# zhufengGNSS/gnss-sdr-1

Measured on AMD Instinct MI355X. Metric: Msamples/s tracked (N-channel multicorrelator, whole job), higher is better.
Workload: dtype f32

## Files before the change

gnss-sdr-1_amd/csrc/trk_closed_loop.hip:

```cpp
#include "gc_internal.h"
#include <algorithm>
#include <cstddef>
#include <cstdlib>
#include "gc_stream.h"
#include "trk_loop_device.hpp"
#include <cstring>
#include <vector>

template <int NTAPS, int THREADS, int FMT, bool DATA, bool HD = false>
__global__ __launch_bounds__(THREADS) void trk_closed_loop_kernel(LoopChan* __restrict__ chans,
    gc_loop_record* __restrict__ recs, int n_epochs, int lds_table_floats, const unsigned long long* __restrict__ limits, int resident)
{
    extern __shared__ float lds[];
    __shared__ LoopChan s;
    __shared__ gc_epoch_params s_p;
    __shared__ float2 s_corr[GC_MAX_TAPS];
    __shared__ int s_go;
    const int ch = blockIdx.x;
    const int tid = threadIdx.x;
    {
        const unsigned* src = reinterpret_cast<const unsigned*>(&chans[ch]);
        unsigned* dst = reinterpret_cast<unsigned*>(&s);
        for (unsigned i = tid; i < sizeof(LoopChan) / 4; i += THREADS) dst[i] = src[i];
    }
    __syncthreads();
    if (s.n_taps != NTAPS)
        {
            for (int e = 0; e < n_epochs; e++)
                {
                    unsigned* w = reinterpret_cast<unsigned*>(&recs[(size_t)ch * n_epochs + e]);
                    for (unsigned i = tid; i < sizeof(gc_loop_record) / 4; i += THREADS) w[i] = 0u;
                }
            return;
        }
    const unsigned long long limit = limits ? limits[ch] : s.chan.n_iq;
    loop_periods<NTAPS, THREADS, FMT, DATA, HD>(s, s_p, s_corr, s_go, lds, &recs[(size_t)ch * n_epochs], n_epochs, lds_table_floats, limit, resident);
    __syncthreads();
    {
        unsigned* dst = reinterpret_cast<unsigned*>(&chans[ch]);
        const unsigned* src = reinterpret_cast<const unsigned*>(&s);
        for (unsigned i = tid; i < sizeof(LoopChan) / 4; i += THREADS) dst[i] = src[i];
    }
}

#ifdef GNSSCORR_EXPERIMENTS
#ifndef LOOP_SLICE_FENCES
#define LOOP_SLICE_FENCES 0
#endif
struct LoopPrep
{
    gc_epoch_params p;
    int go;
    int pad;
};

template <bool HD>
__global__ __launch_bounds__(64) void trk_loop_prepare_kernel(LoopChan* __restrict__ chans, LoopPrep* __restrict__ prep, gc_loop_record* __restrict__ recs, int n_epochs,
    const unsigned long long* __restrict__ limits)
{
    __shared__ LoopChan s;
    __shared__ gc_epoch_params s_p;
    const int ch = blockIdx.x, tid = threadIdx.x;
    {
        const unsigned* src = reinterpret_cast<const unsigned*>(&chans[ch]);
        unsigned* dst = reinterpret_cast<unsigned*>(&s);
        for (unsigned i = tid; i < sizeof(LoopChan) / 4; i += 64) dst[i] = src[i];
    }
    __syncthreads();
    if (s.n_taps == 0) return;
    if (tid == 0)
        {
            const unsigned long long limit = limits ? limits[ch] : s.chan.n_iq;
            const int go = loop_prepare<HD>(s, limit, s_p, &recs[(size_t)ch * n_epochs]);
            prep[ch].p = s_p;
            prep[ch].go = go;
        }
    __syncthreads();
    {
        unsigned* dst = reinterpret_cast<unsigned*>(&chans[ch]);
        const unsigned* src = reinterpret_cast<const unsigned*>(&s);
        for (unsigned i = tid; i < sizeof(LoopChan) / 4; i += 64) dst[i] = src[i];
    }
}

template <int NTAPS, int THREADS, int FMT, bool DATA, bool HD>
__global__ __launch_bounds__(THREADS) void trk_closed_loop_slice_kernel(LoopChan* __restrict__ chans, gc_loop_record* __restrict__ recs, int n_epochs, int e,
    int n_channels, int n_slices, int lds_table_floats, const unsigned long long* __restrict__ limits, LoopPrep* __restrict__ prep, float2* __restrict__ partial,
    unsigned* __restrict__ tickets)
{
    extern __shared__ float lds[];
    __shared__ LoopChan s;
    __shared__ gc_epoch_params s_p;
    __shared__ float2 s_corr[GC_MAX_TAPS];
    __shared__ int s_go, s_last;
    const int tid = threadIdx.x;
    const int x = blockIdx.x & 7, q = blockIdx.x >> 3;
    const int slice = q % n_slices, ch = (q / n_slices) * 8 + x;
    if (ch >= n_channels) return;
    constexpr int NOUT = NTAPS + (DATA ? 1 : 0);
    gc_loop_record* rec = &recs[(size_t)ch * n_epochs + e];
    if (tid == 0)
        {
            s.chan = chans[ch].chan;
            s.n_taps = chans[ch].n_taps;
            s_p = prep[ch].p;
            s_go = prep[ch].go;
        }
    __syncthreads();
    if (s.n_taps != NTAPS)
        {
            if (slice == 0)
                {
                    unsigned* w = reinterpret_cast<unsigned*>(rec);
                    for (unsigned i = tid; i < sizeof(gc_loop_record) / 4; i += THREADS) w[i] = 0u;
                }
            return;
        }
    if (s_go)
        {
            const float2 r = trk_epoch<NTAPS, HD, HD, FMT, false, false, THREADS, DATA, LOOP_PF, false, LOOP_NT != 0, LOOP_WHOLE != 0>(s.chan, s_p, slice, n_slices, lds_table_floats, lds, LOOP_ALIGN_PAIRS);
            if (tid < NOUT) s_corr[tid] = r;
        }
    __syncthreads();
    if (tid == 0)
        {
            float* pv = reinterpret_cast<float*>(partial + ((size_t)ch * n_slices + slice) * GC_MAX_TAPS);
            if (s_go)
                for (int t = 0; t < NOUT; t++)
                    {
                        __hip_atomic_store(pv + 2 * t, s_corr[t].x, __ATOMIC_RELAXED, __HIP_MEMORY_SCOPE_AGENT);
                        __hip_atomic_store(pv + 2 * t + 1, s_corr[t].y, __ATOMIC_RELAXED, __HIP_MEMORY_SCOPE_AGENT);
                    }
#if LOOP_SLICE_FENCES
            __builtin_amdgcn_fence(__ATOMIC_RELEASE, "agent");
#endif
            asm volatile("s_waitcnt vmcnt(0)" ::: "memory");
            const unsigned ticket = __hip_atomic_fetch_add(tickets + ch, 1u, __ATOMIC_RELAXED, __HIP_MEMORY_SCOPE_AGENT);
            s_last = (ticket == (unsigned)n_slices - 1u) ? 1 : 0;
#if LOOP_SLICE_FENCES
            if (s_last) __builtin_amdgcn_fence(__ATOMIC_ACQUIRE, "agent");
#endif
        }
    __syncthreads();
    if (!s_last) return;
    {
        const unsigned* src = reinterpret_cast<const unsigned*>(&chans[ch]);
        unsigned* dst = reinterpret_cast<unsigned*>(&s);
        for (unsigned i = tid; i < sizeof(LoopChan) / 4; i += THREADS) dst[i] = src[i];
    }
    __syncthreads();
    if (tid == 0)
        {
            const unsigned long long limit = limits ? limits[ch] : s.chan.n_iq;
            if (s_go)
                {
                    float2 taps[GC_MAX_TAPS];
                    for (int t = 0; t < NOUT; t++) taps[t] = make_float2(0.f, 0.f);
                    for (int sl = 0; sl < n_slices; sl++)
                        {
                            const float* qv = reinterpret_cast<const float*>(partial + ((size_t)ch * n_slices + sl) * GC_MAX_TAPS);
                            for (int t = 0; t < NOUT; t++)
                                {
                                    taps[t].x += __hip_atomic_load(qv + 2 * t, __ATOMIC_RELAXED, __HIP_MEMORY_SCOPE_AGENT);
                                    taps[t].y += __hip_atomic_load(qv + 2 * t + 1, __ATOMIC_RELAXED, __HIP_MEMORY_SCOPE_AGENT);
                                }
                        }
                    for (int t = 0; t < NOUT; t++) s_corr[t] = taps[t];
                    loop_after_correlation<NTAPS, DATA>(s, s_corr, rec);
                }
            if (e + 1 < n_epochs)
                {
                    const int go = loop_prepare<HD>(s, limit, s_p, rec + 1);
                    prep[ch].p = s_p;
                    prep[ch].go = go;
                }
            __hip_atomic_store(tickets + ch, 0u, __ATOMIC_RELAXED, __HIP_MEMORY_SCOPE_AGENT);
        }
    __syncthreads();
    {
        unsigned* dst = reinterpret_cast<unsigned*>(&chans[ch]);
        const unsigned* src = reinterpret_cast<const unsigned*>(&s);
        for (unsigned i = tid; i < sizeof(LoopChan) / 4; i += THREADS) dst[i] = src[i];
    }
}

#else
struct LoopPrep;
#endif

__global__ void trk_loop_start_kernel(LoopChan* chans, int ch)
{
    if (threadIdx.x == 0 && blockIdx.x == 0) loop_start(chans[ch]);
}

struct gc_trk_loop
{
    gc_ctx* ctx = nullptr;
    gc_ctx_ref ctx_ref;
    int n_channels = 0, max_code_len = 0, n_taps = 0;
    LoopChan* d_chans = nullptr;
    float* d_codes = nullptr;
    float* d_data_codes = nullptr;
    std::vector<LoopSync> sync;
    std::vector<int> data_code_len;
    int pilot = -1;
    int high_dyn = 0;
    int mixed = 0;
    std::vector<int> code_len;
    std::vector<char> track_pilot;
    gc_loop_record* d_recs = nullptr;
    size_t recs_cap = 0;
    int forced_threads = 0;
    int forced_slices = 0;
    LoopPrep* d_prep = nullptr;
    float2* d_slice_partial = nullptr;
    unsigned* d_tickets = nullptr;
    int slice_cap = 0;
    int iq_format = GC_IQ_F32;
    std::vector<char> started;
    std::vector<const void*> iq;
    std::vector<unsigned long long> n_iq;
    std::vector<gc_stream*> streams;
    std::vector<unsigned long long> pos_host;
    std::vector<char> pos_known;
    std::vector<char> idle;
    static constexpr int LIMIT_SLOTS = 8;
    unsigned long long* d_limits[LIMIT_SLOTS] = {};
    unsigned long long* h_limits[LIMIT_SLOTS] = {};
    hipEvent_t limit_done[LIMIT_SLOTS] = {};
    bool limit_used[LIMIT_SLOTS] = {};
    int limit_next = 0;
    hipEvent_t last_launch = nullptr;
    bool launched = false;
};

static hipError_t loop_quiesce(gc_trk_loop* l)
{
    hipError_t e = hipStreamSynchronize(l->ctx->stream);
    if (e == hipSuccess && l->launched) e = hipEventSynchronize(l->last_launch);
    return e;
}

static void loop_free_limits(gc_trk_loop* l)
{
    for (int k = 0; k < gc_trk_loop::LIMIT_SLOTS; k++)
        {
            (void)hipFree(l->d_limits[k]);
            if (l->h_limits[k]) (void)hipHostFree(l->h_limits[k]);
            if (l->limit_done[k]) (void)hipEventDestroy(l->limit_done[k]);
        }
    if (l->last_launch) (void)hipEventDestroy(l->last_launch);
}

extern "C" {

gc_status gc_trk_loop_create(gc_ctx* ctx, int n_channels, int max_code_length, gc_trk_loop** out)
{
    GC_REQUIRE(ctx && out, "gc_trk_loop_create: NULL argument");
    *out = nullptr;
    GC_REQUIRE(n_channels > 0, "gc_trk_loop_create: n_channels must be > 0");
    GC_REQUIRE(max_code_length > 0 && max_code_length + 64 <= 16000, "gc_trk_loop_create: max_code_length must be in 1..%d", 16000 - 64);
    gc_device_guard g(ctx->device);
    gc_trk_loop* l = new gc_trk_loop();
    l->ctx = ctx;
    l->ctx_ref.bind(ctx);
    l->n_channels = n_channels;
    l->max_code_len = max_code_length;
    hipError_t e1 = hipMalloc(&l->d_chans, sizeof(LoopChan) * n_channels);
    hipError_t e2 = hipMalloc(&l->d_codes, sizeof(float) * (size_t)n_channels * max_code_length);
    if (e1 != hipSuccess || e2 != hipSuccess)
// ... 638 lines not shown
```

gnss-sdr-1_amd/csrc/trk_closed_loop_mixed.hip:

```cpp
#include "trk_loop_device.hpp"

template <int THREADS, int FMT, bool HD = false>
__global__ __launch_bounds__(THREADS) void trk_closed_loop_mixed_kernel(LoopChan* __restrict__ chans,
    gc_loop_record* __restrict__ recs, int n_epochs, int lds_table_floats, const unsigned long long* __restrict__ limits, int resident)
{
    extern __shared__ float lds[];
    __shared__ LoopChan s;
    __shared__ gc_epoch_params s_p;
    __shared__ float2 s_corr[GC_MAX_TAPS];
    __shared__ int s_go;
    const int ch = blockIdx.x;
    const int tid = threadIdx.x;
    {
        const unsigned* src = reinterpret_cast<const unsigned*>(&chans[ch]);
        unsigned* dst = reinterpret_cast<unsigned*>(&s);
        for (unsigned i = tid; i < sizeof(LoopChan) / 4; i += THREADS) dst[i] = src[i];
    }
    __syncthreads();
    const int kind = __builtin_amdgcn_readfirstlane(s.n_taps == 0 ? 0 : (s.n_taps == 5 ? 2 : 1) + (s.sync.track_pilot ? 2 : 0));
    gc_loop_record* crec = &recs[(size_t)ch * n_epochs];
    if (kind == 0)
        {
            for (int e = 0; e < n_epochs; e++)
                {
                    unsigned* w = reinterpret_cast<unsigned*>(&crec[e]);
                    for (unsigned i = tid; i < sizeof(gc_loop_record) / 4; i += THREADS) w[i] = 0u;
                }
            return;
        }
    const unsigned long long limit = limits ? limits[ch] : s.chan.n_iq;
    if (kind == 1) loop_periods<3, THREADS, FMT, false, HD>(s, s_p, s_corr, s_go, lds, crec, n_epochs, lds_table_floats, limit, resident);
    else if (kind == 2) loop_periods<5, THREADS, FMT, false, HD>(s, s_p, s_corr, s_go, lds, crec, n_epochs, lds_table_floats, limit, resident);
    else if (kind == 3) loop_periods<3, THREADS, FMT, true, HD>(s, s_p, s_corr, s_go, lds, crec, n_epochs, lds_table_floats, limit, resident);
    else loop_periods<5, THREADS, FMT, true, HD>(s, s_p, s_corr, s_go, lds, crec, n_epochs, lds_table_floats, limit, resident);
    __syncthreads();
    {
        unsigned* dst = reinterpret_cast<unsigned*>(&chans[ch]);
        const unsigned* src = reinterpret_cast<const unsigned*>(&s);
        for (unsigned i = tid; i < sizeof(LoopChan) / 4; i += THREADS) dst[i] = src[i];
    }
}

template <int TH, int FM, bool HD>
static hipError_t loop_launch_mixed_t(LoopChan* d_chans, int n_channels, int n_epochs, gc_loop_record* dev_records, hipStream_t st, int lds_table_floats,
    const unsigned long long* limits, int resident)
{
    const size_t lds_bytes = (size_t)(trk_hdr_floats(TH) + lds_table_floats) * sizeof(float);
    if (lds_bytes > 48 * 1024)
        {
            hipError_t ea = hipFuncSetAttribute(reinterpret_cast<const void*>(&trk_closed_loop_mixed_kernel<TH, FM, HD>), hipFuncAttributeMaxDynamicSharedMemorySize,
                (int)lds_bytes);
            if (ea != hipSuccess) return ea;
        }
    hipLaunchKernelGGL((trk_closed_loop_mixed_kernel<TH, FM, HD>), dim3(n_channels), dim3(TH), lds_bytes, st, d_chans, dev_records, n_epochs,
        lds_table_floats, limits, resident);
    return hipGetLastError();
}

template <int FM>
static hipError_t loop_launch_mixed_f(LoopChan* d_chans, int n_channels, int high_dyn, int threads, int n_epochs, gc_loop_record* dev_records, hipStream_t st,
    int lds_table_floats, const unsigned long long* limits, int resident)
{
    if (high_dyn) return loop_launch_mixed_t<256, FM, true>(d_chans, n_channels, n_epochs, dev_records, st, lds_table_floats, limits, resident);
    if (threads == 1024) return loop_launch_mixed_t<1024, FM, false>(d_chans, n_channels, n_epochs, dev_records, st, lds_table_floats, limits, resident);
    if (threads == 512) return loop_launch_mixed_t<512, FM, false>(d_chans, n_channels, n_epochs, dev_records, st, lds_table_floats, limits, resident);
    return loop_launch_mixed_t<256, FM, false>(d_chans, n_channels, n_epochs, dev_records, st, lds_table_floats, limits, resident);
}

hipError_t loop_launch_mixed(LoopChan* d_chans, int n_channels, int iq_format, int high_dyn, int threads, int n_epochs, gc_loop_record* dev_records,
    hipStream_t st, int lds_table_floats, const unsigned long long* limits, int resident)
{
    if (iq_format == GC_IQ_I16)
        return loop_launch_mixed_f<GC_IQ_I16>(d_chans, n_channels, high_dyn, threads, n_epochs, dev_records, st, lds_table_floats, limits, resident);
    if (iq_format == GC_IQ_I8)
        return loop_launch_mixed_f<GC_IQ_I8>(d_chans, n_channels, high_dyn, threads, n_epochs, dev_records, st, lds_table_floats, limits, resident);
    return loop_launch_mixed_f<GC_IQ_F32>(d_chans, n_channels, high_dyn, threads, n_epochs, dev_records, st, lds_table_floats, limits, resident);
}
```

gnss-sdr-1_amd/csrc/trk_device.hpp:

```cpp
#ifndef TRK_DEVICE_HPP
#define TRK_DEVICE_HPP
#include "gnsscorr.h"
#include "trk_kernels.h"
#include <hip/hip_runtime.h>
#include <type_traits>

#ifndef TRK_THREADS
#define TRK_THREADS 256
#endif
#define TRK_CHUNK (2 * TRK_THREADS)
#define TRK_HDR_FLOATS (TRK_THREADS / 64 * 16)
static constexpr __host__ __device__ int trk_hdr_floats(int threads) { return threads / 64 * 16; }
#define TRK_RESYNC 64
#ifndef TRK_PF
#define TRK_PF 2
#endif
#ifndef TRK_NT
#define TRK_NT 1
#endif
#ifndef TRK_PRELOAD
#define TRK_PRELOAD 0
#endif
#ifndef TRK_ALIGN_PAIRS
#define TRK_ALIGN_PAIRS 8
#endif

static __device__ __forceinline__ int posmod(int i, int L)
{
    int r = i % L;
    return r < 0 ? r + L : r;
}

static __device__ __forceinline__ int chip_index(float step, float nf, float shift, float rem)
{
    float a = step * nf;
    float b = a + shift;
    float c = b - rem;
    return (int)floorf(c);
}

static __device__ __forceinline__ int chip_index_hd(float step, float rate, unsigned n, float shift0, float rem)
{
    float a = step * (float)n;
    float r = rate * (float)(n * n);
    float b = a + r;
    float c = b + shift0;
    float d = c - rem;
    return (int)floorf(d);
}

static __device__ __forceinline__ float wave_sum(float v)
{
#define GC_DPP_ADD(ctrl, row_mask, bank_mask)                                                                    \
    v += __builtin_bit_cast(float, __builtin_amdgcn_update_dpp(0, __builtin_bit_cast(int, v), ctrl, row_mask, bank_mask, false))
    GC_DPP_ADD(0x111, 0xf, 0xf);
    GC_DPP_ADD(0x112, 0xf, 0xf);
    GC_DPP_ADD(0x114, 0xf, 0xe);
    GC_DPP_ADD(0x118, 0xf, 0xc);
    GC_DPP_ADD(0x142, 0xa, 0xf);
    GC_DPP_ADD(0x143, 0xc, 0xf);
#undef GC_DPP_ADD
    return v;
}

static __device__ __forceinline__ int wave_sum_i(int v)
{
#define GC_DPP_ADDI(ctrl, row_mask, bank_mask) v += __builtin_amdgcn_update_dpp(0, v, ctrl, row_mask, bank_mask, false)
    GC_DPP_ADDI(0x111, 0xf, 0xf);
    GC_DPP_ADDI(0x112, 0xf, 0xf);
    GC_DPP_ADDI(0x114, 0xf, 0xe);
    GC_DPP_ADDI(0x118, 0xf, 0xc);
    GC_DPP_ADDI(0x142, 0xa, 0xf);
    GC_DPP_ADDI(0x143, 0xc, 0xf);
#undef GC_DPP_ADDI
    return v;
}

template <bool HDC>
static __device__ __forceinline__ void carrier_at(int n, double theta0, double dtheta, double drate,
    float& zr, float& zi)
{
    double th = fma((double)n, dtheta, theta0);
    if (HDC)
        {
            unsigned m = (n > 0) ? (unsigned)(n - 1) : 0u;
            float e = (float)(m * m);
            th = fma((double)e, drate, th);
        }
    const double inv2pi = 0.15915494309189533577;
    const double twopi = 6.283185307179586477;
    double t = th * inv2pi;
    t -= rint(t);
    float ang = (float)(t * twopi);
    sincosf(ang, &zi, &zr);
}

#define GC_GLOBAL __attribute__((address_space(1)))
typedef float f32x4 __attribute__((ext_vector_type(4)));
typedef float f32x2 __attribute__((ext_vector_type(2)));
typedef short i16x2 __attribute__((ext_vector_type(2)));
typedef short i16x4 __attribute__((ext_vector_type(4)));
typedef signed char i8x2 __attribute__((ext_vector_type(2)));
typedef signed char i8x4 __attribute__((ext_vector_type(4)));

template <int FMT>
struct IqFmt;
template <>
// ... 429 lines not shown
        }
    else
        {
            n_lo = max(c0 * CHUNK - a, 0);
            n_hi = max(min(c1 * CHUNK - a, N) - 1, n_lo);
        }
    float smin = shifts[0], smax = shifts[0];
    if (!HDR)
        {
#pragma unroll
            for (int t = 1; t < NTAPS; t++)
                {
                    smin = fminf(smin, shifts[t]);
                    smax = fmaxf(smax, shifts[t]);
                }
        }
    int lo, hi;
    bool monotone;
    if (HDR)
        {
            lo = chip_index_hd(step, rate, (unsigned)n_lo, shifts[0], rem);
            hi = chip_index_hd(step, rate, (unsigned)n_hi, shifts[0], rem);
            if (DATA)
                {
                    lo = min(lo, chip_index_hd(step, rate, (unsigned)n_lo, shifts[NTAPS / 2], rem));
                    hi = max(hi, chip_index_hd(step, rate, (unsigned)n_hi, shifts[NTAPS / 2], rem));
                }
            monotone = (step > 0.0f) && (rate >= 0.0f) && ((unsigned long long)n_hi * n_hi < 0xffffffffull);
        }
    else
        {
            lo = chip_index(step, (float)n_lo, smin, rem);
            hi = chip_index(step, (float)n_hi, smax, rem);
            monotone = (step >= 0.0f);
        }
    const long long span_ll = (long long)hi - (long long)lo + 1;
    typedef typename std::conditional<CC, f32x2, float>::type chip_t;
    bool windowed = monotone && span_ll > 0 && span_ll * (long long)(sizeof(chip_t) / sizeof(float)) * (DATA ? 2 : 1) <= (long long)lds_table_floats;
    const GC_GLOBAL chip_t* code = (const GC_GLOBAL chip_t*)cd.code;
    chip_t* table_c = reinterpret_cast<chip_t*>(table);
    constexpr int NACC = NTAPS + (DATA ? 1 : 0);
    float* table2 = DATA ? table + (windowed ? (int)span_ll : L) : nullptr;
    const GC_GLOBAL float* code2 = (const GC_GLOBAL float*)cd.code2;
    const bool table_fits = !GTAB || (long long)L * (long long)(sizeof(chip_t) / sizeof(float)) * (DATA ? 2 : 1) <= (long long)lds_table_floats;
    if (resident && !CC)
        {
            windowed = monotone && span_ll > 0 && span_ll <= (long long)L + TRK_RESIDENT_PAD;
            if (windowed) lo -= posmod(lo, L);
            if (DATA) table2 = table + trk_resident_floats(L);
        }
    else if (windowed)
        {
            const int span = (int)span_ll;
            const int cbase = posmod(lo, L);
            if (cbase + span <= 3 * L)
                {
                    for (int k = tid; k < span; k += THREADS)
                        {
                            int i = cbase + k;
                            i = (i >= L) ? i - L : i;
                            i = (i >= L) ? i - L : i;
                            table_c[k] = code[i];
                            if (DATA) table2[k] = code2[i];
                        }
                }
            else
                {
                    for (int k = tid; k < span; k += THREADS)
                        {
                            table_c[k] = code[(cbase + k) % L];
                            if (DATA) table2[k] = code2[(cbase + k) % L];
                        }
                }
        }
    else if (table_fits)
        {
            for (int k = tid; k < L; k += THREADS)
                {
                    table_c[k] = code[k];
                    if (DATA) table2[k] = code2[k];
                }
        }
    __syncthreads();

    float accr[NACC], acci[NACC];
#pragma unroll
    for (int t = 0; t < NACC; t++) accr[t] = acci[t] = 0.0f;

    if constexpr (CHIPS)
        {
            float* scratch = table + ((lds_table_floats + 3) & ~3);
            if (windowed)
                trk_loop_chips<NTAPS, true, THREADS, DATA>(base, table, table2, a, N, V, c0, c1, lo, L, step, rem, shifts, theta0, dtheta, scratch, accr, acci);
            else
                trk_loop_chips<NTAPS, false, THREADS, DATA>(base, table, table2, a, N, V, c0, c1, 0, L, step, rem, shifts, theta0, dtheta, scratch, accr, acci);
        }
    else if (windowed)
        trk_loop<NTAPS, HDR, HDC, true, FMT, CC, SC16, THREADS, DATA, PF, NT, WHOLE>(base, table, a, N, V, c0, c1, lo, L, step, rem, rate, shifts, tap_delay, theta0, dtheta, drate, lnmod, accr, acci, table2, lc0, lc1, pre0, pre1);
    else if (table_fits)
        trk_loop<NTAPS, HDR, HDC, false, FMT, CC, SC16, THREADS, DATA, PF, NT, WHOLE>(base, table, a, N, V, c0, c1, 0, L, step, rem, rate, shifts, tap_delay, theta0, dtheta, drate, lnmod, accr, acci, table2, lc0, lc1, pre0, pre1);
    else if constexpr (GTAB)
        trk_loop<NTAPS, HDR, HDC, false, FMT, CC, SC16, THREADS, DATA, PF, NT, WHOLE>(base, reinterpret_cast<const float*>(cd.code), a, N, V, c0, c1, 0, L, step, rem, rate, shifts, tap_delay, theta0, dtheta, drate, lnmod, accr, acci, cd.code2, lc0, lc1, pre0, pre1);

    __syncthreads();
    const int lane = tid & 63, wave = tid >> 6;
#pragma unroll
    for (int t = 0; t < NACC; t++)
        {
            float sr, si;
            if (SC16)
                {
                    sr = __int_as_float(wave_sum_i(__float_as_int(accr[t])));
                    si = __int_as_float(wave_sum_i(__float_as_int(acci[t])));
                }
            else
                {
                    sr = wave_sum(accr[t]);
                    si = wave_sum(acci[t]);
                }
            if (lane == 63)
                {
                    lds[(wave * NACC + t) * 2 + 0] = sr;
                    lds[(wave * NACC + t) * 2 + 1] = si;
                }
        }
    __syncthreads();
    float2 r = make_float2(0.f, 0.f);
    if (tid < NACC)
        {
            float sr = 0.f, si = 0.f;
#pragma unroll
            for (int w = 0; w < THREADS / 64; w++)
                {
                    if (SC16)
                        {
                            sr = __int_as_float(__float_as_int(sr) + __float_as_int(lds[(w * NACC + tid) * 2 + 0]));
                            si = __int_as_float(__float_as_int(si) + __float_as_int(lds[(w * NACC + tid) * 2 + 1]));
                        }
                    else
                        {
                            sr += lds[(w * NACC + tid) * 2 + 0];
                            si += lds[(w * NACC + tid) * 2 + 1];
                        }
                }
            r = make_float2(sr, si);
        }
    return r;
}

#endif
```

gnss-sdr-1_amd/csrc/trk_loop_device.hpp:

```cpp
#pragma once
#include "gc_internal.h"
#include "trk_device.hpp"

#define LOOP_MAX_CN0 64
#ifndef LOOP_NT
#define LOOP_NT 0
#endif
#ifndef LOOP_WHOLE
#define LOOP_WHOLE 0
#endif
#ifndef LOOP_ALIGN_PAIRS
#define LOOP_ALIGN_PAIRS 1
#endif
#ifndef LOOP_PF
#define LOOP_PF 2
#endif
#define LOOP_MAX_SMOOTHER 16
#define LOOP_PI_2 6.283185307179586

struct DevLoopFilter
{
    float b[4], a[3];
    int nb, na;
    float in[4], out[4];
    int idx;
};

struct DevPll
{
    int order;
    float w, x, a2, a3, b3, w0p, w0p2, w0p3, w0f, w0f2;
};

struct LoopSync
{
    int extend_symbols, track_pilot, symbols_per_bit, secondary_len, preamble_len;
    float bit_sync_min_time_s, pll_bw_narrow_hz, dll_bw_narrow_hz, el_narrow_chips, vel_narrow_chips;
    unsigned sec_ones[4];
    unsigned pre_plus[6];
};

struct LoopChan
{
    gc_loop_conf conf;
    LoopSync sync;
    unsigned hist[6];
    int hist_count;
    float2 accu[5];
    float2 prompt_data;
    int current_symbol, extend_count;
    double carr_hist[2 * LOOP_MAX_SMOOTHER][2], code_hist[2 * LOOP_MAX_SMOOTHER][2];
    int carr_hist_n, code_hist_n;
    double carrier_phase_rate_step_rad, code_phase_rate_step_chips;
    TrkChan chan;
    int n_taps;
    int state;
    int cloop, pull_in_transitory;
    unsigned long long pos;
    unsigned long long sample_counter;
    unsigned long long acq_sample_stamp;
    double acq_code_phase_samples, acq_carrier_doppler_hz;
    double carrier_doppler_hz, code_freq_chips;
    double carrier_phase_step_rad, code_phase_step_chips;
    double rem_code_phase_samples, rem_code_phase_chips, acc_carrier_phase_rad;
    float rem_carr_phase_rad;
    int current_prn_length_samples;
    double current_correlation_time_s;
    double carr_phase_error_hz, carr_freq_error_hz, carr_error_filt_hz, code_error_chips, code_error_filt_chips;
    float2 P_accu_old;
    DevLoopFilter dll;
    DevPll pll;
    float2 prompt_buffer[LOOP_MAX_CN0];
    int cn0_estimation_counter, carrier_lock_fail_counter;
    double carrier_lock_test, cn0_db_hz;
    int lost_lock_events;
};

static __device__ __forceinline__ void dll_design(DevLoopFilter& f, int order, float bw, float T)
{
    const float zeta = 1.0 / sqrt(2.0);
    float g1, g2, g3, wn;
    f.nb = f.na = 0;
    switch (order)
        {
        case 1:
            wn = bw * 4.0;
            g1 = wn;
            f.b[0] = g1;
            f.nb = 1;
            break;
        case 3:
            {
                wn = bw / 0.7845;
                const float a3 = 1.1, b3 = 2.4;
                g1 = wn * wn * wn;
                g2 = a3 * wn * wn;
                g3 = b3 * wn;
                f.b[0] = g3 + T / 2.0 * (g2 + T / 2.0 * g1);
                f.b[1] = g1 * T * T / 2.0 - 2.0 * g3;
                f.b[2] = g3 + T / 2.0 * (-g2 + T / 2.0 * g1);
// ... 259 lines not shown

static __device__ __forceinline__ void loop_update_tracking_vars(LoopChan& s)
{
    const gc_loop_conf& c = s.conf;
    const int sl = (int)c.high_dyn_smoother_length;
    const double T_prn_samples = (1.0 / s.code_freq_chips) * (double)c.code_length_chips * c.fs_in;
    const double K_blk_samples = T_prn_samples + s.rem_code_phase_samples;
    s.current_prn_length_samples = (int)floor(K_blk_samples);
    s.carrier_phase_step_rad = LOOP_PI_2 * s.carrier_doppler_hz / c.fs_in;
    const double n = (double)s.current_prn_length_samples;
    if (sl > 0) s.carrier_phase_rate_step_rad = loop_smoothed_rate(s.carr_hist, s.carr_hist_n, sl, s.carrier_phase_step_rad, n, s.carrier_phase_rate_step_rad);
    s.rem_carr_phase_rad += (float)(s.carrier_phase_step_rad * n + 0.5 * s.carrier_phase_rate_step_rad * n * n);
    s.rem_carr_phase_rad = fmodf(s.rem_carr_phase_rad, (float)LOOP_PI_2);
    s.acc_carrier_phase_rad -= (s.carrier_phase_step_rad * n + 0.5 * s.carrier_phase_rate_step_rad * n * n);
    s.code_phase_step_chips = s.code_freq_chips / c.fs_in;
    if (sl > 0) s.code_phase_rate_step_chips = loop_smoothed_rate(s.code_hist, s.code_hist_n, sl, s.code_phase_step_chips, n, s.code_phase_rate_step_chips);
    s.rem_code_phase_samples = K_blk_samples - n;
    s.rem_code_phase_chips = s.code_freq_chips * s.rem_code_phase_samples / c.fs_in;
}

static __device__ __forceinline__ void loop_save_correlation_results(LoopChan& s, const float2* taps, bool veml)
{
    const LoopSync& y = s.sync;
    float sign = 1.0f;
    if (y.secondary_len > 0)
        {
            const int bit = y.secondary_len - 1 - s.current_symbol;
            if ((y.sec_ones[bit >> 5] >> (bit & 31)) & 1u) sign = -1.0f;
            s.current_symbol = (s.current_symbol + 1) % y.secondary_len;
        }
    else
        {
            s.current_symbol++;
            s.current_symbol = y.symbols_per_bit > 0 ? s.current_symbol % y.symbols_per_bit : 0;
        }
    for (int t = 0; t < 5; t++)
        {
            if (!veml && (t == 0 || t == 4)) continue;
            const float2 v = taps[veml ? t : t - 1];
            if (sign > 0.0f)
                {
                    s.accu[t].x += v.x;
                    s.accu[t].y += v.y;
                }
            else
                {
                    s.accu[t].x -= v.x;
                    s.accu[t].y -= v.y;
                }
        }
    s.cloop = y.track_pilot ? 0 : 1;
}

static __device__ __forceinline__ bool loop_push_and_match(LoopChan& s, float prompt_re, int len, const unsigned* pattern, bool either_polarity)
{
    const unsigned neg = prompt_re < 0.0f ? 1u : 0u;
    for (int w = 5; w > 0; w--) s.hist[w] = (s.hist[w] << 1) | (s.hist[w - 1] >> 31);
    s.hist[0] = (s.hist[0] << 1) | neg;
    if (s.hist_count < len) s.hist_count++;
    if (s.hist_count < len) return false;
    int diff = 0;
    for (int w = 0; w * 32 < len; w++)
        {
            const int nb = min(32, len - w * 32);
            const unsigned mask = nb == 32 ? 0xffffffffu : ((1u << nb) - 1u);
            diff += __popc((s.hist[w] ^ pattern[w]) & mask);
        }
    return either_polarity ? (diff == 0 || diff == len) : diff == len;
}

static __device__ __forceinline__ void loop_write_record(const LoopChan& s, gc_loop_record* rec, int valid, int integrating, int extend_count)
{
    for (int t = 0; t < 5; t++)
        {
            rec->accu[2 * t] = s.accu[t].x;
            rec->accu[2 * t + 1] = s.accu[t].y;
        }
    rec->extend_count = extend_count;
    rec->integrating = integrating;
    rec->valid = valid;
}

template <int NTAPS, bool DATA>
static __device__ __forceinline__ void loop_after_correlation(LoopChan& s, const float2* taps, gc_loop_record* rec)
{
    const gc_loop_conf& c = s.conf;
    const LoopSync& y = s.sync;
    const bool veml = NTAPS == 5;
    const float2 P = taps[NTAPS / 2];
    {
        unsigned* w = reinterpret_cast<unsigned*>(rec);
        for (unsigned i = 0; i < sizeof(gc_loop_record) / 4; i++) w[i] = 0u;
    }
    for (int t = 0; t < NTAPS; t++)
        {
            rec->corr[2 * t] = taps[t].x;
            rec->corr[2 * t + 1] = taps[t].y;
        }
    s.prompt_data = DATA ? taps[NTAPS] : P;
    const int ext = y.extend_symbols > 1 ? y.extend_symbols : 1;
    if (s.state == 2)
        {
            for (int t = 0; t < 5; t++) s.accu[t] = make_float2(0.f, 0.f);
            for (int t = 0; t < NTAPS; t++) s.accu[veml ? t : t + 1] = taps[t];
            if (!loop_lock_status(s, c.code_period_s))
                {
                    loop_clear_tracking_vars(s);
                    s.state = 0;
                    loop_write_record(s, rec, 0, 0, 0);
                }
            else
                {
                    loop_run_dll_pll(s, veml);
                    loop_update_tracking_vars(s);
                    loop_write_record(s, rec, 1, 0, s.extend_count);
                    bool next_state;
                    if (y.secondary_len > 0)
                        {
                            next_state = loop_push_and_match(s, P.x, y.secondary_len, y.sec_ones, true);
                        }
                    else if (y.symbols_per_bit > 1)
                        {
                            next_state = false;
                            const float t_trk = (float)((double)(float)(s.sample_counter - s.acq_sample_stamp) / c.fs_in);
                            if (t_trk > y.bit_sync_min_time_s && y.preamble_len > 0)
                                {
                                    next_state = loop_push_and_match(s, P.x, y.preamble_len, y.pre_plus, false);
                                }
                        }
                    else
                        next_state = true;
                    if (next_state)
                        {
                            for (int t = 0; t < 5; t++) s.accu[t] = make_float2(0.f, 0.f);
                            s.hist_count = 0;
                            for (int i = 0; i < 6; i++) s.hist[i] = 0u;
                            s.current_symbol = 0;
                            if (ext > 1)
                                {
                                    s.extend_count = 0;
                                    s.current_correlation_time_s = (double)((float)ext * (float)c.code_period_s);
                                    s.state = 3;
                                    dll_design(s.dll, c.dll_filter_order, y.dll_bw_narrow_hz, (float)s.current_correlation_time_s);
                                    pll_retune(s.pll, c.fll_bw_hz, y.pll_bw_narrow_hz, c.pll_filter_order);
                                    const float spc = (float)c.code_samples_per_chip;
                                    if (veml)
                                        {
                                            s.chan.shifts[0] = -y.vel_narrow_chips * spc;
                                            s.chan.shifts[1] = -y.el_narrow_chips * spc;
                                            s.chan.shifts[3] = y.el_narrow_chips * spc;
                                            s.chan.shifts[4] = y.vel_narrow_chips * spc;
                                        }
                                    else
                                        {
                                            s.chan.shifts[0] = -y.el_narrow_chips * spc;
                                            s.chan.shifts[2] = y.el_narrow_chips * spc;
                                        }
                                }
                            else
                                s.state = 4;
                        }
                }
        }
    else if (s.state == 3)
        {
            loop_update_tracking_vars(s);
            loop_save_correlation_results(s, taps, veml);
            s.extend_count++;
            if (s.extend_count == ext - 1)
                {
                    s.extend_count = 0;
                    s.state = 4;
                }
            loop_write_record(s, rec, 1, 1, s.extend_count);
        }
    else
        {
            loop_save_correlation_results(s, taps, veml);
            if (!loop_lock_status(s, c.code_period_s * (double)ext))
                {
                    loop_clear_tracking_vars(s);
                    s.state = 0;
                    loop_write_record(s, rec, 0, 0, 0);
                }
            else
                {
                    loop_run_dll_pll(s, veml);
                    loop_update_tracking_vars(s);
                    loop_write_record(s, rec, 1, 0, s.extend_count);
                    for (int t = 0; t < 5; t++) s.accu[t] = make_float2(0.f, 0.f);
                    if (ext > 1) s.state = 3;
                }
        }
    s.sample_counter += (unsigned long long)s.current_prn_length_samples;
    s.pos += (unsigned long long)s.current_prn_length_samples;
    rec->prompt_data[0] = s.prompt_data.x;
    rec->prompt_data[1] = s.prompt_data.y;
    rec->sample_counter = s.sample_counter;
    rec->acc_carrier_phase_rad = s.acc_carrier_phase_rad;
    rec->rem_code_phase_samples = s.rem_code_phase_samples;
    rec->carrier_doppler_hz = (float)s.carrier_doppler_hz;
    rec->code_freq_chips = (float)s.code_freq_chips;
    rec->carr_phase_error_hz = (float)s.carr_phase_error_hz;
    rec->carr_error_filt_hz = (float)s.carr_error_filt_hz;
    rec->code_error_chips = (float)s.code_error_chips;
    rec->code_error_filt_chips = (float)s.code_error_filt_chips;
    rec->cn0_db_hz = (float)s.cn0_db_hz;
    rec->carrier_lock_test = (float)s.carrier_lock_test;
    rec->state = s.state;
    rec->current_prn_length_samples = s.current_prn_length_samples;
}

template <bool HD>
static __device__ __forceinline__ int loop_prepare(LoopChan& s, unsigned long long limit, gc_epoch_params& s_p, gc_loop_record* rec)
{
    const gc_loop_conf& c = s.conf;
    int go = 1;
    if (s.pull_in_transitory)
        {
            if (c.pull_in_time_s < (s.sample_counter - s.acq_sample_stamp) / (unsigned long long)(int)c.fs_in) s.pull_in_transitory = 0;
        }
    if (s.state == 1)
        {
            const long long acq_trk_diff_samples = (long long)s.sample_counter - (long long)s.acq_sample_stamp;
            const double delta = (double)acq_trk_diff_samples - s.acq_code_phase_samples;
            s.code_freq_chips = c.code_chip_rate_hz;
            s.code_phase_step_chips = s.code_freq_chips / c.fs_in;
            const double T_prn_mod_samples = (1.0 / s.code_freq_chips) * (double)c.code_length_chips * c.fs_in;
            s.acq_code_phase_samples = T_prn_mod_samples - fmod(delta, T_prn_mod_samples);
            s.current_prn_length_samples = (int)round(T_prn_mod_samples);
            const int samples_offset = (int)round(s.acq_code_phase_samples);
            s.acc_carrier_phase_rad -= s.carrier_phase_step_rad * (double)samples_offset;
            s.state = 2;
            s.sample_counter += samples_offset;
            s.pos += samples_offset;
        }
    if (s.state < 2 || s.pos + c.vector_length > limit) go = 0;
    if (go)
        {
            const float spc = (float)c.code_samples_per_chip;
            const float rem_carr = s.rem_carr_phase_rad;
            const float pstep = (float)s.carrier_phase_step_rad;
            s_p.sample_offset = s.pos;
            s_p.phase0_re = cosf(rem_carr);
            s_p.phase0_im = -sinf(rem_carr);
            s_p.phase_inc_re = cosf(pstep);
            s_p.phase_inc_im = -sinf(pstep);
            const float prate = HD ? (float)s.carrier_phase_rate_step_rad : 0.0f;
            s_p.phase_rate_re = cosf(prate);
            s_p.phase_rate_im = -sinf(prate);
            s_p.rem_code_phase_chips = (float)s.rem_code_phase_chips * spc;
            s_p.code_phase_step_chips = (float)s.code_phase_step_chips * spc;
            s_p.code_phase_rate_step_chips = HD ? (float)s.code_phase_rate_step_chips * spc : 0.0f;
            s_p.n_samples = (int)c.vector_length;
        }
    else
        {
            unsigned* w = reinterpret_cast<unsigned*>(rec);
            for (unsigned i = 0; i < sizeof(gc_loop_record) / 4; i++) w[i] = 0u;
            rec->state = s.state;
            rec->sample_counter = s.sample_counter;
        }
    return go;
}

template <int NTAPS, int THREADS, int FMT, bool DATA, bool HD>
static __device__ __forceinline__ void loop_periods(LoopChan& s, gc_epoch_params& s_p, float2* s_corr, int& s_go, float* lds, gc_loop_record* crec,
    int n_epochs, int lds_table_floats, unsigned long long limit, int resident)
{
    const int tid = threadIdx.x;
    if (resident)
        {
            trk_fill_resident<THREADS>(lds, s.chan.code, DATA ? s.chan.code2 : nullptr, s.chan.code_len);
            __syncthreads();
        }

    for (int e = 0; e < n_epochs; e++)
        {
            gc_loop_record* rec = &crec[e];
            if (tid == 0)
                {
                    const int go = loop_prepare<HD>(s, limit, s_p, rec);
                    s_go = go;
                }
            __syncthreads();
            if (!s_go) continue;

            const float2 r = trk_epoch<NTAPS, HD, HD, FMT, false, false, THREADS, DATA, LOOP_PF, false, LOOP_NT != 0, LOOP_WHOLE != 0>(s.chan, s_p, 0, 1, lds_table_floats, lds, LOOP_ALIGN_PAIRS, resident != 0);
            if (tid < NTAPS + (DATA ? 1 : 0)) s_corr[tid] = r;
            __syncthreads();

            if (tid == 0) loop_after_correlation<NTAPS, DATA>(s, s_corr, rec);
        }
}

hipError_t loop_launch_mixed(LoopChan* d_chans, int n_channels, int iq_format, int high_dyn, int threads, int n_epochs, gc_loop_record* dev_records,
    hipStream_t st, int lds_table_floats, const unsigned long long* limits, int resident);
```

Measured before the change: 793,000.

## Stage loop records in LDS and overlap next-epoch prepare with state update

The per-epoch closed-loop bookkeeping is split into a state machine, record-tail writing and prepare steps. Records are staged in a double-buffered shared-memory slot and copied to global memory in parallel by wave 1 one epoch later, instead of thread 0 zeroing and writing each record serially. The next epoch's prepare now runs right after the state update, with its sin/cos work spread across lanes, so it shares a barrier with the state machine rather than needing its own. This shortens the single-thread serial tail between correlation passes. The risk is that the record tail now reads channel state after the next prepare may have changed it, and timing-stamp instrumentation is added behind a compile flag.

Result: no change. 792,300 (-0.1%).

```diff
diff --git a/gnss-sdr-1_amd/csrc/trk_closed_loop.hip b/gnss-sdr-1_amd/csrc/trk_closed_loop.hip
--- a/gnss-sdr-1_amd/csrc/trk_closed_loop.hip
+++ b/gnss-sdr-1_amd/csrc/trk_closed_loop.hip
@@ -16,6 +16,7 @@
     __shared__ gc_epoch_params s_p;
     __shared__ float2 s_corr[GC_MAX_TAPS];
     __shared__ int s_go;
+    __shared__ gc_loop_record s_rec[2];
     const int ch = blockIdx.x;
     const int tid = threadIdx.x;
     {
@@ -34,7 +35,7 @@
             return;
         }
     const unsigned long long limit = limits ? limits[ch] : s.chan.n_iq;
-    loop_periods<NTAPS, THREADS, FMT, DATA, HD>(s, s_p, s_corr, s_go, lds, &recs[(size_t)ch * n_epochs], n_epochs, lds_table_floats, limit, resident);
+    loop_periods<NTAPS, THREADS, FMT, DATA, HD>(s, s_p, s_corr, s_go, s_rec, lds, &recs[(size_t)ch * n_epochs], n_epochs, lds_table_floats, limit, resident);
     __syncthreads();
     {
         unsigned* dst = reinterpret_cast<unsigned*>(&chans[ch]);
@@ -186,6 +187,14 @@
 
 #else
 struct LoopPrep;
+#endif
+
+#ifdef GNSSCORR_LOOP_STAMPS
+extern "C" int gc_trk_loop_debug_set_stamps(void* dev_buf)
+{
+    unsigned long long* p = static_cast<unsigned long long*>(dev_buf);
+    return (int)hipMemcpyToSymbol(HIP_SYMBOL(g_loop_stamps), &p, sizeof p);
+}
 #endif
 
 __global__ void trk_loop_start_kernel(LoopChan* chans, int ch)
diff --git a/gnss-sdr-1_amd/csrc/trk_closed_loop_mixed.hip b/gnss-sdr-1_amd/csrc/trk_closed_loop_mixed.hip
--- a/gnss-sdr-1_amd/csrc/trk_closed_loop_mixed.hip
+++ b/gnss-sdr-1_amd/csrc/trk_closed_loop_mixed.hip
@@ -9,6 +9,7 @@
     __shared__ gc_epoch_params s_p;
     __shared__ float2 s_corr[GC_MAX_TAPS];
     __shared__ int s_go;
+    __shared__ gc_loop_record s_rec[2];
     const int ch = blockIdx.x;
     const int tid = threadIdx.x;
     {
@@ -29,10 +30,10 @@
             return;
         }
     const unsigned long long limit = limits ? limits[ch] : s.chan.n_iq;
-    if (kind == 1) loop_periods<3, THREADS, FMT, false, HD>(s, s_p, s_corr, s_go, lds, crec, n_epochs, lds_table_floats, limit, resident);
-    else if (kind == 2) loop_periods<5, THREADS, FMT, false, HD>(s, s_p, s_corr, s_go, lds, crec, n_epochs, lds_table_floats, limit, resident);
-    else if (kind == 3) loop_periods<3, THREADS, FMT, true, HD>(s, s_p, s_corr, s_go, lds, crec, n_epochs, lds_table_floats, limit, resident);
-    else loop_periods<5, THREADS, FMT, true, HD>(s, s_p, s_corr, s_go, lds, crec, n_epochs, lds_table_floats, limit, resident);
+    if (kind == 1) loop_periods<3, THREADS, FMT, false, HD>(s, s_p, s_corr, s_go, s_rec, lds, crec, n_epochs, lds_table_floats, limit, resident);
+    else if (kind == 2) loop_periods<5, THREADS, FMT, false, HD>(s, s_p, s_corr, s_go, s_rec, lds, crec, n_epochs, lds_table_floats, limit, resident);
+    else if (kind == 3) loop_periods<3, THREADS, FMT, true, HD>(s, s_p, s_corr, s_go, s_rec, lds, crec, n_epochs, lds_table_floats, limit, resident);
+    else loop_periods<5, THREADS, FMT, true, HD>(s, s_p, s_corr, s_go, s_rec, lds, crec, n_epochs, lds_table_floats, limit, resident);
     __syncthreads();
     {
         unsigned* dst = reinterpret_cast<unsigned*>(&chans[ch]);
diff --git a/gnss-sdr-1_amd/csrc/trk_device.hpp b/gnss-sdr-1_amd/csrc/trk_device.hpp
--- a/gnss-sdr-1_amd/csrc/trk_device.hpp
+++ b/gnss-sdr-1_amd/csrc/trk_device.hpp
@@ -23,6 +23,22 @@
 #endif
 #ifndef TRK_ALIGN_PAIRS
 #define TRK_ALIGN_PAIRS 8
+#endif
+
+#ifdef GNSSCORR_LOOP_STAMPS
+static __shared__ unsigned long long trk_stamps[3];
+#define TRK_STAMP(k)                                                          \
+    do                                                                        \
+        {                                                                     \
+            if (threadIdx.x == 0) trk_stamps[k] = __builtin_amdgcn_s_memtime(); \
+        }                                                                     \
+    while (0)
+#else
+#define TRK_STAMP(k) \
+    do               \
+        {            \
+        }            \
+    while (0)
 #endif
 
 static __device__ __forceinline__ int posmod(int i, int L)
@@ -618,6 +634,7 @@
                 }
         }
     __syncthreads();
+    TRK_STAMP(0);
 
     float accr[NACC], acci[NACC];
 #pragma unroll
@@ -639,6 +656,7 @@
         trk_loop<NTAPS, HDR, HDC, false, FMT, CC, SC16, THREADS, DATA, PF, NT, WHOLE>(base, reinterpret_cast<const float*>(cd.code), a, N, V, c0, c1, 0, L, step, rem, rate, shifts, tap_delay, theta0, dtheta, drate, lnmod, accr, acci, cd.code2, lc0, lc1, pre0, pre1);
 
     __syncthreads();
+    TRK_STAMP(1);
     const int lane = tid & 63, wave = tid >> 6;
 #pragma unroll
     for (int t = 0; t < NACC; t++)
@@ -681,6 +699,7 @@
                 }
             r = make_float2(sr, si);
         }
+    TRK_STAMP(2);
     return r;
 }
 
diff --git a/gnss-sdr-1_amd/csrc/trk_loop_device.hpp b/gnss-sdr-1_amd/csrc/trk_loop_device.hpp
--- a/gnss-sdr-1_amd/csrc/trk_loop_device.hpp
+++ b/gnss-sdr-1_amd/csrc/trk_loop_device.hpp
@@ -16,6 +16,25 @@
 #define LOOP_PF 2
 #endif
 #define LOOP_MAX_SMOOTHER 16
+#define LOOP_REC_DWORDS ((int)(sizeof(gc_loop_record) / 4))
+
+#ifdef GNSSCORR_LOOP_STAMPS
+#define LOOP_STAMP_SLOTS 10
+static __device__ unsigned long long* g_loop_stamps;
+static __shared__ unsigned long long* s_stamp_row;
+#define LOOP_STAMP(k)                                                         \
+    do                                                                        \
+        {                                                                     \
+            if (s_stamp_row) s_stamp_row[k] = __builtin_amdgcn_s_memtime();   \
+        }                                                                     \
+    while (0)
+#else
+#define LOOP_STAMP(k) \
+    do                \
+        {             \
+        }             \
+    while (0)
+#endif
 #define LOOP_PI_2 6.283185307179586
 
 struct DevLoopFilter
@@ -441,21 +460,12 @@
 }
 
 template <int NTAPS, bool DATA>
-static __device__ __forceinline__ void loop_after_correlation(LoopChan& s, const float2* taps, gc_loop_record* rec)
+static __device__ __forceinline__ void loop_state_machine(LoopChan& s, const float2* taps, gc_loop_record* rec)
 {
     const gc_loop_conf& c = s.conf;
     const LoopSync& y = s.sync;
     const bool veml = NTAPS == 5;
     const float2 P = taps[NTAPS / 2];
-    {
-        unsigned* w = reinterpret_cast<unsigned*>(rec);
-        for (unsigned i = 0; i < sizeof(gc_loop_record) / 4; i++) w[i] = 0u;
-    }
-    for (int t = 0; t < NTAPS; t++)
-        {
-            rec->corr[2 * t] = taps[t].x;
-            rec->corr[2 * t + 1] = taps[t].y;
-        }
     s.prompt_data = DATA ? taps[NTAPS] : P;
     const int ext = y.extend_symbols > 1 ? y.extend_symbols : 1;
     if (s.state == 2)
@@ -553,6 +563,10 @@
         }
     s.sample_counter += (unsigned long long)s.current_prn_length_samples;
     s.pos += (unsigned long long)s.current_prn_length_samples;
+}
+
+static __device__ __forceinline__ void loop_record_tail(const LoopChan& s, gc_loop_record* rec)
+{
     rec->prompt_data[0] = s.prompt_data.x;
     rec->prompt_data[1] = s.prompt_data.y;
     rec->sample_counter = s.sample_counter;
@@ -570,8 +584,23 @@
     rec->current_prn_length_samples = s.current_prn_length_samples;
 }
 
-template <bool HD>
-static __device__ __forceinline__ int loop_prepare(LoopChan& s, unsigned long long limit, gc_epoch_params& s_p, gc_loop_record* rec)
+template <int NTAPS, bool DATA>
+static __device__ __forceinline__ void loop_after_correlation(LoopChan& s, const float2* taps, gc_loop_record* rec)
+{
+    {
+        unsigned* w = reinterpret_cast<unsigned*>(rec);
+        for (unsigned i = 0; i < sizeof(gc_loop_record) / 4; i++) w[i] = 0u;
+    }
+    for (int t = 0; t < NTAPS; t++)
+        {
+            rec->corr[2 * t] = taps[t].x;
+            rec->corr[2 * t + 1] = taps[t].y;
+        }
+    loop_state_machine<NTAPS, DATA>(s, taps, rec);
+    loop_record_tail(s, rec);
+}
+
+static __device__ __forceinline__ int loop_prepare_state(LoopChan& s, unsigned long long limit)
 {
     const gc_loop_conf& c = s.conf;
     int go = 1;
@@ -595,12 +624,29 @@
             s.pos += samples_offset;
         }
     if (s.state < 2 || s.pos + c.vector_length > limit) go = 0;
+    return go;
+}
+
+template <bool HD>
+static __device__ __forceinline__ void loop_prepare_scalars(const LoopChan& s, gc_epoch_params& s_p)
+{
+    const gc_loop_conf& c = s.conf;
+    const float spc = (float)c.code_samples_per_chip;
+    s_p.sample_offset = s.pos;
+    s_p.rem_code_phase_chips = (float)s.rem_code_phase_chips * spc;
+    s_p.code_phase_step_chips = (float)s.code_phase_step_chips * spc;
+    s_p.code_phase_rate_step_chips = HD ? (float)s.code_phase_rate_step_chips * spc : 0.0f;
+    s_p.n_samples = (int)c.vector_length;
+}
+
+template <bool HD>
+static __device__ __forceinline__ int loop_prepare(LoopChan& s, unsigned long long limit, gc_epoch_params& s_p, gc_loop_record* rec)
+{
+    const int go = loop_prepare_state(s, limit);
     if (go)
         {
-            const float spc = (float)c.code_samples_per_chip;
             const float rem_carr = s.rem_carr_phase_rad;
             const float pstep = (float)s.carrier_phase_step_rad;
-            s_p.sample_offset = s.pos;
             s_p.phase0_re = cosf(rem_carr);
             s_p.phase0_im = -sinf(rem_carr);
             s_p.phase_inc_re = cosf(pstep);
@@ -608,10 +654,7 @@
             const float prate = HD ? (float)s.carrier_phase_rate_step_rad : 0.0f;
             s_p.phase_rate_re = cosf(prate);
             s_p.phase_rate_im = -sinf(prate);
-            s_p.rem_code_phase_chips = (float)s.rem_code_phase_chips * spc;
-            s_p.code_phase_step_chips = (float)s.code_phase_step_chips * spc;
-            s_p.code_phase_rate_step_chips = HD ? (float)s.code_phase_rate_step_chips * spc : 0.0f;
-            s_p.n_samples = (int)c.vector_length;
+            loop_prepare_scalars<HD>(s, s_p);
         }
     else
         {
@@ -623,34 +666,154 @@
     return go;
 }
 
+template <bool HD>
+static __device__ __forceinline__ void loop_prepare_wave(LoopChan& s, unsigned long long limit, gc_epoch_params& s_p, int& s_go)
+{
+    const int lane = threadIdx.x;
+    int go = 0;
+    float a0 = 0.0f, a1 = 0.0f, a2 = 0.0f;
+    if (lane == 0)
+        {
+            go = loop_prepare_state(s, limit);
+            if (go)
+                {
+                    a0 = s.rem_carr_phase_rad;
+                    a1 = (float)s.carrier_phase_step_rad;
+                    a2 = HD ? (float)s.carrier_phase_rate_step_rad : 0.0f;
+                    loop_prepare_scalars<HD>(s, s_p);
+                }
+            s_go = go;
+        }
+    go = __builtin_amdgcn_readfirstlane(go);
+    if (!go) return;
+    a0 = __int_as_float(__builtin_amdgcn_readfirstlane(__float_as_int(a0)));
+    a1 = __int_as_float(__builtin_amdgcn_readfirstlane(__float_as_int(a1)));
+    a2 = __int_as_float(__builtin_amdgcn_readfirstlane(__float_as_int(a2)));
+    if (lane < (HD ? 3 : 2))
+        {
+            const float ang = lane == 0 ? a0 : (lane == 1 ? a1 : a2);
+            const float re = cosf(ang), im = -sinf(ang);
+            if (lane == 0)
+                {
+                    s_p.phase0_re = re;
+                    s_p.phase0_im = im;
+                    if (!HD)
+                        {
+                            s_p.phase_rate_re = cosf(0.0f);
+                            s_p.phase_rate_im = -sinf(0.0f);
+                        }
+                }
+            else if (lane == 1)
+                {
+                    s_p.phase_inc_re = re;
+                    s_p.phase_inc_im = im;
+                }
+            else
+                {
+                    s_p.phase_rate_re = re;
+                    s_p.phase_rate_im = im;
+                }
+        }
+}
+
+template <int WAVE>
+static __device__ __forceinline__ void loop_record_out(gc_loop_record* slot, gc_loop_record* dst)
+{
+    const int i = (int)threadIdx.x - 64 * WAVE;
+    if (i >= 0 && i < LOOP_REC_DWORDS)
+        {
+            unsigned* w = reinterpret_cast<unsigned*>(slot);
+            const unsigned v = w[i];
+            w[i] = 0u;
+            reinterpret_cast<unsigned*>(dst)[i] = v;
+        }
+}
+
 template <int NTAPS, int THREADS, int FMT, bool DATA, bool HD>
-static __device__ __forceinline__ void loop_periods(LoopChan& s, gc_epoch_params& s_p, float2* s_corr, int& s_go, float* lds, gc_loop_record* crec,
-    int n_epochs, int lds_table_floats, unsigned long long limit, int resident)
-{
+static __device__ __forceinline__ void loop_periods(LoopChan& s, gc_epoch_params& s_p, float2* s_corr, int& s_go, gc_loop_record* s_rec, float* lds,
+    gc_loop_record* crec, int n_epochs, int lds_table_floats, unsigned long long limit, int resident)
+{
+    static_assert(THREADS >= 128 && 2 * LOOP_REC_DWORDS <= THREADS, "wave 1 copies records out");
     const int tid = threadIdx.x;
-    if (resident)
-        {
-            trk_fill_resident<THREADS>(lds, s.chan.code, DATA ? s.chan.code2 : nullptr, s.chan.code_len);
-            __syncthreads();
-        }
-
+    if (tid < 2 * LOOP_REC_DWORDS) reinterpret_cast<unsigned*>(s_rec)[tid] = 0u;
+    if (resident) trk_fill_resident<THREADS>(lds, s.chan.code, DATA ? s.chan.code2 : nullptr, s.chan.code_len);
+#ifdef GNSSCORR_LOOP_STAMPS
+    if (tid == 0)
+        {
+            s_stamp_row = g_loop_stamps ? g_loop_stamps + (size_t)blockIdx.x * n_epochs * LOOP_STAMP_SLOTS : nullptr;
+            if (s_stamp_row) s_stamp_row[8] = __builtin_amdgcn_s_memrealtime(), s_stamp_row[9] = 1ull;
+            LOOP_STAMP(0);
+            LOOP_STAMP(6);
+        }
+#endif
+    if (tid < 64) loop_prepare_wave<HD>(s, limit, s_p, s_go);
+    __syncthreads();
+
+    int pending = -1;
     for (int e = 0; e < n_epochs; e++)
         {
-            gc_loop_record* rec = &crec[e];
-            if (tid == 0)
-                {
-                    const int go = loop_prepare<HD>(s, limit, s_p, rec);
-                    s_go = go;
-                }
-            __syncthreads();
-            if (!s_go) continue;
+            gc_loop_record* slot = &s_rec[e & 1];
+            if (!s_go)
+                {
+                    if (tid == 0)
+                        {
+                            slot->state = s.state;
+                            slot->sample_counter = s.sample_counter;
+                        }
+                    __syncthreads();
+                    if (pending >= 0) loop_record_out<1>(&s_rec[pending & 1], &crec[pending]);
+                    loop_record_out<0>(slot, &crec[e]);
+                    pending = -1;
+                    if (e + 1 < n_epochs && tid < 64) loop_prepare_wave<HD>(s, limit, s_p, s_go);
+                    __syncthreads();
+                    continue;
+                }
 
             const float2 r = trk_epoch<NTAPS, HD, HD, FMT, false, false, THREADS, DATA, LOOP_PF, false, LOOP_NT != 0, LOOP_WHOLE != 0>(s.chan, s_p, 0, 1, lds_table_floats, lds, LOOP_ALIGN_PAIRS, resident != 0);
             if (tid < NTAPS + (DATA ? 1 : 0)) s_corr[tid] = r;
             __syncthreads();
 
-            if (tid == 0) loop_after_correlation<NTAPS, DATA>(s, s_corr, rec);
-        }
+            if (pending >= 0) loop_record_out<1>(&s_rec[pending & 1], &crec[pending]);
+            if (tid < 64)
+                {
+                    if (tid == 0)
+                        {
+#ifdef GNSSCORR_LOOP_STAMPS
+                            if (s_stamp_row)
+                                for (int k = 0; k < 3; k++) s_stamp_row[2 + k] = trk_stamps[k];
+#endif
+                            loop_state_machine<NTAPS, DATA>(s, s_corr, slot);
+                            LOOP_STAMP(5);
+                        }
+                    if (e + 1 < n_epochs) loop_prepare_wave<HD>(s, limit, s_p, s_go);
+                    if (tid == 0) LOOP_STAMP(1);
+                }
+            __syncthreads();
+            if (tid == 0)
+                {
+#ifdef GNSSCORR_LOOP_STAMPS
+                    if (s_stamp_row && e + 1 < n_epochs)
+                        {
+                            s_stamp_row += LOOP_STAMP_SLOTS;
+                            s_stamp_row[8] = __builtin_amdgcn_s_memrealtime();
+                            s_stamp_row[9] = 1ull;
+                            LOOP_STAMP(0);
+                        }
+#endif
+                    for (int t = 0; t < NTAPS; t++)
+                        {
+                            slot->corr[2 * t] = s_corr[t].x;
+                            slot->corr[2 * t + 1] = s_corr[t].y;
+                        }
+                    loop_record_tail(s, slot);
+#ifdef GNSSCORR_LOOP_STAMPS
+                    if (e + 1 < n_epochs) LOOP_STAMP(6);
+#endif
+                }
+            pending = e;
+        }
+    __syncthreads();
+    if (pending >= 0) loop_record_out<1>(&s_rec[pending & 1], &crec[pending]);
 }
 
 hipError_t loop_launch_mixed(LoopChan* d_chans, int n_channels, int iq_format, int high_dyn, int threads, int n_epochs, gc_loop_record* dev_records,
```
